# szpiech/garlic

Measured on AMD Instinct MI355X. Metric: LOD-windows/sec (SNPs x inds / winsize), higher is better.
Workload: dtype f64

## Files before the change

### garlic_amd/csrc/garlic_hip.hip

```cpp
#include "../../include/garlic_hip.h"
#include "lod_kernels.hpp"
#include "variant_kernels.hpp"
#include "ld_kernels.hpp"
#include "ld_multi_kernel.hpp"
#include "tgls_ring_kernel.hpp"
#include "tgls_wide_kernel.hpp"
#include "tgls_feed_kernel.hpp"
#include "tgls_feed_multi_kernel.hpp"
#include "wlod_strip_kernel.hpp"
#include "wlod_small_kernel.hpp"
#include "coverage_kernel.hpp"
#include "roh_segments_kernel.hpp"
#include "feed_kernel.hpp"
#include "wlod_feed_kernel.hpp"
#include "feed_sort_kernel.hpp"
#include "kde_kernels.hpp"
#include "kde_multi_kernels.hpp"
#include "kde_part_set_kernels.hpp"
#include "gmm_kernels.hpp"
#include "feature_kernels.hpp"
#include "../host/kde_select.hpp"
#include "../host/kde_parts.hpp"
#include "../host/chain_order.hpp"
#include "bed_kernels.hpp"
// ... 225 lines not shown
    {
        if (p) (void)score_free(ctx, p);
        p = nullptr;
    }
};


struct garlic_panel {
    garlic_ctx *ctx = nullptr;
    int32_t nchr = 0;
    int32_t nind = 0;
    int64_t nloci = 0;
    int64_t nind_pad = 0;
    int64_t nwordrows = 0;
    std::vector<int32_t> chr_nloci;
    std::vector<int64_t> chr_off;
    std::vector<int32_t> pos, cs, ce;
    std::vector<double> gpos, freq;
    bool have_map = false, have_freq = false, have_geno = false, have_gpos = false;
    DevBuf<uint32_t> d_packed;
    DevBuf<int32_t> d_pos, d_cs, d_ce;
    DevBuf<int64_t> d_chr_off;
    DevBuf<double> d_tab;
    bool tab_valid = false;
    double tab_error = 0;
    double tab_min = 0, tabgl_min = 0, glterms_min = 0;
    bool tab_all_finite = false;
    bool seg_valid = false;
    int32_t seg_max_gap = 0;
    std::vector<int64_t> boundaries;
    DevBuf<int32_t> d_blk_counts, d_blk_offsets, d_total;
    DevBuf<int64_t> d_boundaries;
    DevBuf<ChainItem> d_items;
    DevBuf<FeedItem> d_feed_items;
    DevBuf<FillItem> d_fill;
    DevBuf<int32_t> d_counter;
    DevBuf<ChrDev> d_chrs;
    DevBuf<int16_t> d_stage16;
    DevBuf<int32_t> d_bed_word_rows;
    DevBuf<int64_t> d_row_counts;
    bool have_gl = false;
    std::vector<double> gl_values;
    std::unordered_map<uint64_t, int> gl_code;
    DevBuf<uint8_t> d_codes;
    DevBuf<double> d_tabgl;
    bool tabgl_valid = false;
    DevBuf<double> d_glterms;
    bool glterms_valid = false, glterms_scaled = false;
    int32_t glterms_M = 0;
    double glterms_mu = 0.0;
    int64_t terms_budget = 0;
    DevBuf<double> d_slab[2];
    hipStream_t slab_stream = nullptr;
    hipEvent_t ev_slab_begin = nullptr, ev_slab_built[2] = {}, ev_slab_read[2] = {};
    DevBuf<int32_t> d_slab_queues;
    int32_t last_slab_blocks = 0, last_n_slabs = 0;

    int tabgl_ncodes = 0;
    bool gl_cont = false;
    DevBuf<double> d_glval;
    bool gl_vals_dropped = false;
    bool gl_cover_required = false;
    std::vector<uint8_t> gl_cover;
    DevBuf<double> d_freq;
    bool dfreq_valid = false;
    int gl_terms_by = 0;
// ... 1412 lines not shown
    const bool ring_patch = !getenv("GARLIC_WLOD_GL_NO_PATCH");
    const int strip_waves = (W + 15 - 16 * WS_WAVES <= 16 || getenv("GARLIC_WLOD_STRIP_NARROW_ONLY")) ? WS_WAVES : WS_WAVES_WIDE;
    const bool wlod_gl_strip = wlod_gl_ring && W + 15 - 16 * strip_waves <= 16 && !getenv("GARLIC_WLOD_GL_NO_STRIP");
    f.strip_waves = strip_waves;
    f.use_patch = wlod_gl_ring ? ring_patch : wlod_use_patch;
    f.tile_lds = wlod_gl_ring ? WLOD_GL_RING_OFF + (size_t)WLOD_WAVES * GARLIC_WLOD_GL_RING_ROWS * WAVE * 8
                              : wlod_rows + 16 + (wlod_use_patch ? wlod_patch : 0);
    f.strip_force_rerun = wlod_gl_strip && getenv("GARLIC_WLOD_STRIP_FORCE_RERUN") != nullptr;
    f.family = wlod_stream                            ? Family::wlod_stream
               : wlod_small                           ? Family::wlod_small_tiles
               : wlod_gl_strip                        ? Family::wlod_strip
               : wlod_gl_ring                         ? Family::wlod_glring
               : f.wlod_gl                            ? Family::wlod_tile_gl
               : !getenv("GARLIC_WLOD_ONE_BLOCK")     ? Family::wlod_tile2
                                                      : Family::wlod_tile;
    return GARLIC_OK;
}

void finish_form(const garlic_panel *p, const LodCall &c, const Layout &L, const double *d_out, LodForm &f)
{
    f.aligned16 = (c.pitch_align % 2 == 0) && ((reinterpret_cast<uintptr_t>(d_out) & 15) == 0);
    if (f.family == Family::wlod_stream && !f.aligned16) f.family = Family::wlod_small_tiles;
    f.strip_three = f.family == Family::wlod_strip && f.strip_waves != WS_WAVES_WIDE && f.aligned16 && !f.cov_bits &&
                    !getenv("GARLIC_WLOD_STRIP_TWO_PER_CU");
    for (int k = 0; f.strip_three && k < p->nchr; k++) f.strip_three = L.pitch[k] * 8 < ((int64_t)1 << 32);
}

using Plan = garlic_panel::Plan;

struct LodWork {
    std::vector<Run> runs;
    std::vector<FillItem> fill;
    std::vector<ChainItem> items;
    std::vector<FeedItem> feed_items;
    std::vector<ChrDev> chrs;
    std::vector<uint8_t> valid;
    std::vector<int2> tiles, segs;
    std::vector<WlodStrip> strips;
    std::vector<int32_t> feed_blocks;
};

int chain_workers(const garlic_ctx *ctx, size_t n_items)
{
    int workers = ctx->n_cu;
    if (const char *e = getenv("GARLIC_WORKERS")) workers = std::max(1, atoi(e));
    return std::min<int>(workers, (int)n_items);
}

int plan_lod(garlic_panel *p, const LodCall &c, const LodForm &form, const Layout &L, const garlic_panel::PlanKey &key, LodWork &w, Plan &plan)
{
    plan = Plan{false, key};
    const int nblk = (c.ind_count + WAVE - 1) / WAVE;
    int rc;
    p->plan.valid = false;
    plan_runs(p, c.W, w.runs, w.fill, plan.n_valid);
    const std::vector<int> order = longest_first(w.runs);
    w.items.reserve(w.runs.size() * nblk);
    const bool wlod_slabs = form.slab_blocks && (form.wlod_tuned || form.family == Family::wlod_feed);
    const int per_list = form.slab_blocks ? form.slab_blocks : std::max(nblk, 1);
    for (int k0 = 0; k0 < nblk && (!w.runs.empty() || wlod_slabs); ) {
        if (c.blocks && !(*c.blocks)[(size_t)k0]) { k0++; continue; }
        const int k1 = std::min(nblk, k0 + per_list);
        const size_t item0 = w.items.size();
        for (size_t i = 0; i < order.size(); i++) {
            const Run &r = w.runs[order[i]];
            for (int k = k0; k < k1; k++)
                if (!c.blocks || (*c.blocks)[(size_t)k]) w.items.push_back(ChainItem{r.chr, r.a, r.b, k * WAVE});
        }
        if (form.slab_blocks) plan.slabs.push_back(Plan::Slab{c.ind_begin / WAVE + k0, c.ind_begin / WAVE + k1, item0, w.items.size() - item0});
        k0 = k1;
    }
    if (form.family == Family::chain && !form.slab_blocks) {
        std::vector<int32_t> len(w.items.size());
        for (size_t i = 0; i < len.size(); i++) len[i] = w.items[i].b - w.items[i].a + 1;
        const std::vector<int> at = garlic_host::chainOrder(len, chain_workers(p->ctx, len.size()));
        std::vector<ChainItem> sorted(w.items.size());
        for (size_t i = 0; i < at.size(); i++) sorted[i] = w.items[(size_t)at[i]];
        w.items.swap(sorted);
    }
    if (form.family == Family::feed) {
        std::vector<int32_t> col0(w.runs.size());
        for (size_t i = 0; i < w.runs.size(); i++) {
            const int32_t s = (w.runs[i].a + c.thin_step - 1) / c.thin_step;
            col0[i] = (int64_t)s * c.thin_step <= w.runs[i].b ? s : -1;
        }
        build_feed_items(w.runs, order, c.blocks, nblk, col0, w.feed_items);
        plan.n_feed_items = w.feed_items.size();
    }
    w.chrs.resize(p->nchr);
    for (int k = 0; k < p->nchr; k++)
        w.chrs[k] = ChrDev{p->chr_off[k], L.base[k], L.pitch[k], p->chr_nloci[k],
                           (c.pitch_align >= 2 && 64 * L.pitch[k] * 8 + 512 < ((int64_t)1 << 32)) ? 1 : 0};
    plan.n_items = w.items.size();
    plan.n_fill = w.fill.size();
    plan.n_runs = (int64_t)w.runs.size();
    if (!p->d_counter.p) {
        if ((rc = p->d_counter.reserve(8))) return rc;
        HIP_TRY(hipMemsetAsync(p->d_counter.p, 0, 8 * sizeof(int32_t), p->ctx->stream));
    }
    if (form.wlod_tuned || form.family == Family::wlod_feed) {
        w.valid.assign((size_t)p->nloci, 0);
        for (const Run &r : w.runs)
            memset(w.valid.data() + p->chr_off[r.chr] + r.a, 1, (size_t)(r.b - r.a + 1));
    }
    if (form.family == Family::wlod_feed) {
        for (int k = 0; k < p->nchr; k++) {
            const int32_t cols = (int32_t)(((int64_t)p->chr_nloci[k] + c.thin_step - 1) / c.thin_step);
            for (int32_t c0 = 0; c0 < cols; c0 += WFD_COLS) w.tiles.push_back(make_int2(k, c0));
        }
        plan.n_tiles = (int32_t)w.tiles.size();
        for (int k = 0; k < nblk; k++)
            if (!c.blocks || (*c.blocks)[(size_t)k]) w.feed_blocks.push_back(k);
        plan.n_feed_blocks = (int32_t)w.feed_blocks.size();
        size_t at = 0;
        for (Plan::Slab &sl : plan.slabs) {
            sl.fb0 = (int32_t)at;
            while (at < w.feed_blocks.size() && w.feed_blocks[at] < sl.b1) at++;
            sl.n_fb = (int32_t)at - sl.fb0;
        }
    }
    if (form.wlod_tuned) {
        for (int k = 0; k < p->nchr; k++)
            for (int s0 = 0; s0 < p->chr_nloci[k]; s0 += TILE) w.tiles.push_back(make_int2(k, s0));
        plan.n_tiles = (int32_t)w.tiles.size();
        for (int k = 0; k < p->nchr; k++)
// ... 157 lines not shown
        HIP_TRY(hipLaunchKernel(fn, dim3((sa.n_work + 7u) / 8u * 8u), dim3((form.strip_waves + 1) * WAVE), kargs, strip_lds, s));
        if (form.strip_force_rerun) HIP_TRY(hipMemsetAsync(p->d_counter.p + 3, 1, sizeof(int32_t), s));
        a.run_if = p->d_counter.p + 3;
        a.rerun_count = p->d_counter.p + 4;
        p->reruns_stale = true;
    }
    const void *fn = wlod_tile_fn(form.family, form.wlod_gl, form.aligned16);
    if (form.tile_lds > LDS_DEFAULT_MAX) HIP_TRY(hipFuncSetAttribute(fn, hipFuncAttributeMaxDynamicSharedMemorySize, (int)form.tile_lds));
    void *kargs[] = {(void *)&a_packed, (void *)&a_wtab, (void *)&a_skew, (void *)&d_out, (void *)&a};
    HIP_TRY(hipLaunchKernel(fn, dim3((a.n_work + 7u) / 8u * 8u), wl_block, kargs, form.tile_lds, s));
    return GARLIC_OK;
}

bool chain_takes_fill(const LodForm &form, const Plan &plan, Family family)
{
    return family == Family::chain && plan.n_items && plan.n_fill && !form.wlod_tuned && !form.cov_bits;
}

int launch_chain(garlic_panel *p, const LodCall &c, const LodForm &form, Plan &plan, const LodWork *fresh, int workers, double *d_out)
{
    garlic_ctx *ctx = p->ctx;
    ItemTrace trace;
    if (form.family == Family::feed && plan.n_feed_items) {
        FeedArgs f{p->d_packed.p, p->d_tab.p, p->d_feed_items.p, p->d_chrs.p, d_out, nullptr, p->nwordrows, c.ind_begin, c.ind_count, c.W,
                   (int32_t)plan.n_feed_items, c.thin_step, form.feed_asm ? 1 : 0, p->d_counter.p, nullptr};
        f.trace = trace.begin(8, plan.n_feed_items, "\n", ctx->stream);
        int grid = (int)std::min<size_t>(plan.n_feed_items, (size_t)ctx->n_cu * std::max(1, plan.feed_per_cu)), rc;
        if (fresh && (rc = feed_grid(ctx, fresh->feed_items, &grid, &plan.feed_per_cu))) return rc;
        void *kargs[] = {(void *)&f};
        HIP_TRY(hipLaunchKernel((const void *)lod_feed_kernel, dim3((unsigned)grid), dim3(FEED_G * WAVE), kargs, 0, ctx->stream));
    } else {
        ChainArgs a{p->d_packed.p, p->d_tab.p, p->d_items.p,     p->d_chrs.p,          d_out, p->nind_pad, p->nwordrows,
                    c.ind_begin,   c.ind_count, c.W,             (int32_t)plan.n_items, p->d_counter.p, nullptr,
                    nullptr,       0};
        if (chain_takes_fill(form, plan, form.family)) {
            a.fill = p->d_fill.p;
            a.n_fill = (int32_t)plan.n_fill;
        }
        a.trace = trace.begin(4, plan.n_items, " 0\n", ctx->stream);
        if (form.aligned16)
            hipLaunchKernelGGL((lod_chain_kernel<true>), dim3((unsigned)workers), dim3(CHAIN_THREADS), 0, ctx->stream, a);
        else
            hipLaunchKernelGGL((lod_chain_kernel<false>), dim3((unsigned)workers), dim3(CHAIN_THREADS), 0, ctx->stream, a);
    }
    trace.write(ctx->stream);
    return GARLIC_OK;
}

template <class Chains>
int for_each_tgls_slab(garlic_panel *p, const std::vector<Plan::Slab> &slabs, int32_t slab_blocks, Chains chains, bool scaled = false)
{
    garlic_ctx *ctx = p->ctx;
    hipStream_t s = ctx->stream;
    const int64_t rows = GOFF + p->nloci + GPAD_BACK;
    const size_t n_slabs = slabs.size();
    int rc;
    p->last_slab_blocks = slab_blocks;
    p->last_n_slabs = (int32_t)n_slabs;
    if (!n_slabs) return GARLIC_OK;
    if (!p->slab_stream) {
        HIP_TRY(hipStreamCreateWithFlags(&p->slab_stream, hipStreamNonBlocking));
        for (hipEvent_t *ev : {&p->ev_slab_begin, &p->ev_slab_built[0], &p->ev_slab_built[1], &p->ev_slab_read[0], &p->ev_slab_read[1]})
            HIP_TRY(hipEventCreateWithFlags(ev, hipEventDisableTiming));
    }
    for (int q = 0; q < 2; q++) {
        size_t blocks = 0;
        for (size_t k = (size_t)q; k < n_slabs; k += 2) blocks = std::max(blocks, (size_t)(slabs[k].b1 - slabs[k].b0));
// ... 114 lines not shown
    return GARLIC_OK;
}

int launch_wlod_feed(garlic_panel *p, const LodCall &c, const LodForm &form, const Plan &plan, double *d_out, const WlodTerms &t,
                     int32_t fb0, int32_t n_fb)
{
    const int nquad = (n_fb + WFD_WAVES - 1) / WFD_WAVES;
    WlodFeedArgs a{p->d_packed.p, form.wlod_gl ? t.terms : p->d_wtab.p, p->d_skew.p + SKEW_FRONT, p->d_valid.p, p->d_chrs.p,
                   p->d_tiles.p, p->d_feed_blocks.p + fb0, d_out, p->nwordrows, GOFF + p->nloci + GPAD_BACK, c.ind_count, c.W, c.thin_step,
                   n_fb, nquad, (uint32_t)((int64_t)plan.n_tiles * nquad), t.blk0};
    if (!a.n_work) return GARLIC_OK;
    if (form.wlod_gl) hipLaunchKernelGGL(wlod_feed_kernel<true>, dim3(a.n_work), dim3(WFD_WAVES * WAVE), 0, p->ctx->stream, a);
    else hipLaunchKernelGGL(wlod_feed_kernel<false>, dim3(a.n_work), dim3(WFD_WAVES * WAVE), 0, p->ctx->stream, a);
    return GARLIC_OK;
}

int launch_wlod_slabs(garlic_panel *p, const LodCall &c, const LodForm &form, const Plan &plan, double *d_out)
{
    return for_each_tgls_slab(p, plan.slabs, form.slab_blocks, [&](size_t k, const double *terms) {
        const Plan::Slab &sl = plan.slabs[k];
        const WlodTerms t = wlod_terms_slab(c, sl, terms);
        if (form.family == Family::wlod_feed) return launch_wlod_feed(p, c, form, plan, d_out, t, sl.fb0, sl.n_fb);
        return launch_wlod(p, c, form, plan, d_out, t);
    }, true);
}

int enqueue_lod(garlic_panel *p, const LodCall &c, const LodForm &form, const Layout &L, Plan &plan, const LodWork *fresh,
                double *d_out, Family family, bool one_kernel = false)
{
    garlic_ctx *ctx = p->ctx;
    hipStream_t s = ctx->stream;
    int rc = GARLIC_OK;
    if (!one_kernel) HIP_TRY(hipEventRecord(ctx->ev_begin, s));
    if (fresh && ((rc = p->d_chrs.put(fresh->chrs, s)) || (rc = p->d_items.put(fresh->items, s)) || (rc = p->d_fill.put(fresh->fill, s)) ||
                  (rc = p->d_feed_items.put(fresh->feed_items, s)) || (rc = p->d_valid.put(fresh->valid, s)) ||
                  (rc = p->d_tiles.put(fresh->tiles, s)) || (rc = p->d_segs.put(fresh->segs, s)) || (rc = p->d_strips.put(fresh->strips, s)) ||
                  (rc = p->d_feed_blocks.put(fresh->feed_blocks, s))))
        return rc;
    if (family == Family::feed || family == Family::tgls_feed) {
        hipLaunchKernelGGL(fill_value_kernel, dim3(1024), dim3(256), 0, s, d_out, L.total, MISSING_D);
    } else if (plan.n_fill && !form.wlod_tuned && family != Family::wlod_feed && !form.cov_bits &&
               !chain_takes_fill(form, plan, family)) {
        dim3 grid((unsigned)plan.n_fill, (unsigned)((c.ind_count + FILL_ROWS - 1) / FILL_ROWS));
        hipLaunchKernelGGL(fill_missing_kernel, grid, dim3(256), 0, s, p->d_fill.p, p->d_chrs.p, c.ind_count, d_out);
    }
    if (plan.n_items && (fresh || c.mode != MODE_LOD)) HIP_TRY(hipMemsetAsync(p->d_counter.p, 0, 2 * sizeof(int32_t), s));
    p->stats_slot = (int)(ctx->n_calls % garlic_ctx::HIST);
    HIP_TRY(hist_mark(ctx, false));
    const int workers = chain_workers(ctx, plan.n_items);
    if (form.wlod_tuned || plan.n_items || family == Family::wlod_feed)
        switch (family) {
        case Family::chain:
        case Family::feed: rc = launch_chain(p, c, form, plan, fresh, workers, d_out); break;
        case Family::exact:
            hipLaunchKernelGGL(lod_chain_exact_kernel, dim3((unsigned)plan.n_items), dim3(WAVE), 0, s, variant_args(p, c, form, d_out),
                               (int)plan.n_items);
            break;
        case Family::tgls_ring:
        case Family::tgls_feed:
        case Family::tgls_terms:
        case Family::tgls_lookup: rc = launch_tgls(p, c, form, plan, workers, d_out); break;
        case Family::wlod_generic: rc = launch_generic_wlod(p, c, form, plan, d_out); break;
        case Family::wlod_feed:
            rc = form.slab_blocks ? launch_wlod_slabs(p, c, form, plan, d_out)
                                  : launch_wlod_feed(p, c, form, plan, d_out, wlod_terms_whole(p, c), 0, plan.n_feed_blocks);
            break;
        default:
// ... 5186 lines not shown
```

### garlic_amd/csrc/lod_kernels.hpp

```cpp
#pragma once
#include <hip/hip_runtime.h>
#include <stdint.h>

#include "chain_loop_gfx950.inc"

namespace garlic {

constexpr int WAVE = 64;
constexpr int TILE = 32;
constexpr int TPITCH = 34;
constexpr int GOFF = 32;
constexpr int GPAD_CHAIN = 32 * GARLIC_CHAIN_NSLOT + 48 * GARLIC_CHAIN_CHROWS + 64;
constexpr int GPAD_BACK = GPAD_CHAIN > 4160 ? GPAD_CHAIN : 4160;
constexpr double MISSING_D = -9999.0;

struct ChrDev {
    int64_t loc_base;
    int64_t out_base;
    int64_t out_pitch;
    int32_t nloci;
    int32_t fast;
};

struct ChainItem {
    int32_t chr;
    int32_t a;
    int32_t b;
    int32_t ind0;
};

struct FillItem {
    int32_t chr;
    int32_t lo;
    int32_t hi;
    int32_t pad;
};

__device__ __host__ __forceinline__ int64_t packed_index(int64_t w, int64_t col, int64_t nwordrows)
{
    return (((col >> 6) * nwordrows + w) << 6) + (col & 63);
}

__global__ void pack_genotypes_kernel(const int16_t *__restrict__ geno, int64_t ld,
                                      int64_t locus_begin, int64_t locus_count, int32_t nind,
                                      int64_t nind_pad, int64_t nwordrows,
                                      uint32_t *__restrict__ packed, int64_t word_lo,
                                      int64_t word_hi)
{
    int64_t ind = (int64_t)blockIdx.x * blockDim.x + threadIdx.x;
    int64_t w = word_lo + blockIdx.y;
    if (ind >= nind_pad || w >= word_hi) return;
    uint32_t *dst = packed + packed_index(w, ind, nwordrows);
    uint32_t word = *dst;
    if (ind >= nind) { *dst = 0xFFFFFFFFu; return; }
    int64_t g0 = w * 16 - GOFF;
#pragma unroll
    for (int q = 0; q < 16; q++) {
        int64_t l = g0 + q - locus_begin;
        if (l >= 0 && l < locus_count) {
            int v = geno[l * ld + ind];
            uint32_t code = (v == 0) ? 0u : (v == 1) ? 1u : (v == 2) ? 2u : 3u;
            word = (word & ~(3u << (2 * q))) | (code << (2 * q));
// ... 139 lines not shown
__device__ __forceinline__ void fill_rows(const FillItem &it, const ChrDev &c, int row0, int32_t nind, double *out,
                                          int wave, int nwaves, int lane)
{
    for (int r = row0 + wave; r < row0 + FILL_ROWS && r < nind; r += nwaves) {
        double *row = out + c.out_base + (int64_t)r * c.out_pitch;
        for (int l = it.lo + lane; l < it.hi; l += WAVE) row[l] = MISSING_D;
    }
}

__global__ void __launch_bounds__(256)
fill_missing_kernel(const FillItem *items, const ChrDev *chrs, int32_t nind, double *out)
{
    FillItem it = items[blockIdx.x];
    ChrDev c = chrs[it.chr];
    fill_rows(it, c, blockIdx.y * FILL_ROWS, nind, out, threadIdx.x >> 6, 4, threadIdx.x & 63);
}

struct ChainArgs {
    const uint32_t *packed;
    const double *tab;
    const ChainItem *items;
    const ChrDev *chrs;
    double *out;
    int64_t nind_pad;
    int64_t nwordrows;
    int32_t ind_begin;
    int32_t ind_count;
    int32_t winsize;
    int32_t n_items;
    int32_t *next_item;
    int64_t *trace;
    const FillItem *fill;
    int32_t n_fill;
};

__device__ __forceinline__ void chain_fill_share(const ChainArgs &p, int wave, int first, int lane)
{
    const int groups = (p.ind_count + FILL_ROWS - 1) / FILL_ROWS;
    const int64_t units = (int64_t)p.n_fill * groups;
    for (int64_t u = blockIdx.x; u < units; u += gridDim.x) {
        const FillItem it = p.fill[u / groups];
        const ChrDev c = p.chrs[it.chr];
        fill_rows(it, c, (int)(u % groups) * FILL_ROWS, p.ind_count, p.out, wave - first, 4 - first, lane);
    }
}

constexpr uint32_t SLOT_BYTES = 3072;
constexpr uint32_t SL_LW1 = 0, SL_LW2 = 256, SL_TW1 = 512, SL_TW2 = 768;
constexpr uint32_t SL_LTAB = 1024, SL_TTAB = 2048;
constexpr uint32_t LDS_ITEM = 3072;
constexpr uint32_t LDS_TILE = GARLIC_CHAIN_LDS_TILE0;
constexpr uint32_t LDS_BYTES = GARLIC_CHAIN_LDS_TOTAL;
constexpr int CHAIN_THREADS = 256;

struct Streams {
    int64_t lead_w, trail_w;
    const double *lead_tab, *trail_tab;
    int sh_lead, sh_trail;
};

__device__ __forceinline__ void advance(Streams &st)
{
    st.lead_w += 2; st.trail_w += 2;
    st.lead_tab += 4 * TILE; st.trail_tab += 4 * TILE;
}

__device__ __forceinline__ void fill_regs(unsigned char *smem, const Streams &st,
                                          const uint32_t *gcol, int lane)
{
    const uint32_t l1 = gcol[(st.lead_w + 1) * WAVE], l2 = gcol[(st.lead_w + 2) * WAVE];
    const uint32_t t1 = gcol[(st.trail_w + 1) * WAVE], t2 = gcol[(st.trail_w + 2) * WAVE];
    const double2 tl = reinterpret_cast<const double2 *>(st.lead_tab)[lane];
    const double2 tt = reinterpret_cast<const double2 *>(st.trail_tab)[lane];
    *reinterpret_cast<uint32_t *>(smem + SL_LW1 + lane * 4) = l1;
    *reinterpret_cast<uint32_t *>(smem + SL_LW2 + lane * 4) = l2;
    *reinterpret_cast<uint32_t *>(smem + SL_TW1 + lane * 4) = t1;
    *reinterpret_cast<uint32_t *>(smem + SL_TW2 + lane * 4) = t2;
    *reinterpret_cast<double2 *>(smem + SL_LTAB + lane * 16) = tl;
    *reinterpret_cast<double2 *>(smem + SL_TTAB + lane * 16) = tt;
}

struct TileBits {
    uint32_t lead_lo, lead_hi, trail_lo, trail_hi;
};

template <int SLOT>
__device__ __forceinline__ TileBits tile_consume(const unsigned char *smem, uint32_t &lc,
                                                 uint32_t &tc, const Streams &st, int lane)
{
    const unsigned char *slot = smem + SLOT * SLOT_BYTES;
    const uint32_t l1 = *reinterpret_cast<const uint32_t *>(slot + SL_LW1 + lane * 4);
    const uint32_t l2 = *reinterpret_cast<const uint32_t *>(slot + SL_LW2 + lane * 4);
    const uint32_t t1 = *reinterpret_cast<const uint32_t *>(slot + SL_TW1 + lane * 4);
    const uint32_t t2 = *reinterpret_cast<const uint32_t *>(slot + SL_TW2 + lane * 4);
    TileBits tb;
    tb.lead_lo = __builtin_amdgcn_alignbit(l1, lc, st.sh_lead);
    tb.lead_hi = __builtin_amdgcn_alignbit(l2, l1, st.sh_lead);
    tb.trail_lo = __builtin_amdgcn_alignbit(t1, tc, st.sh_trail);
    tb.trail_hi = __builtin_amdgcn_alignbit(t2, t1, st.sh_trail);
    lc = l2;
    tc = t2;
    return tb;
}

template <bool EDGE, int SLOT>
__device__ __forceinline__ void tile_steps(const unsigned char *smem, unsigned char *tile,
                                           double &acc, const TileBits &tb, int s0, int a, int b,
                                           int lane)
{
    const unsigned char *slot = smem + SLOT * SLOT_BYTES;
    const uint32_t tile_lane = (uint32_t)lane * (TPITCH * 8);
#pragma unroll
// ... 10 lines not shown
            if (!(s >= a && s <= b)) t_in = 0.0;
        }
        acc = (acc - t_out) + t_in;
        *reinterpret_cast<double *>(tile + tile_lane + j * 8) = acc;
    }
}

template <bool EDGE, bool ALIGNED16>
__device__ __forceinline__ void tile_store(const unsigned char *tile, int s0, int a, int b, int lane,
                                           int rows_valid, double *out_tile, int64_t pitch)
{
    const int rsub = lane >> 4, csub = lane & 15;
#pragma unroll
    for (int q = 0; q < WAVE / 4; q++) {
        const int qe = (4 * q < rows_valid) ? q : 0;
        const int re = min(rsub, rows_valid - 1 - 4 * qe);
        const double2 v = *reinterpret_cast<const double2 *>(
            tile + (uint32_t)(4 * qe + re) * (TPITCH * 8) + csub * 16);
        char *base = reinterpret_cast<char *>(out_tile + (int64_t)(4 * qe) * pitch);
        const uint32_t off = (uint32_t)re * (uint32_t)(pitch * 8) + (uint32_t)csub * 16u;
        double *dst = reinterpret_cast<double *>(base + off);
        if (EDGE) {
            const int s = s0 + 2 * csub;
            if (s >= a && s <= b) dst[0] = v.x;
            if (s + 1 >= a && s + 1 <= b) dst[1] = v.y;
        } else if (!ALIGNED16) {
            dst[0] = v.x;
            dst[1] = v.y;
        } else {
            *reinterpret_cast<double2 *>(dst) = v;
        }
    }
}

__global__ void __launch_bounds__(256) fill_value_kernel(double *dst, int64_t n, double value)
{
    for (int64_t i = (int64_t)blockIdx.x * blockDim.x + threadIdx.x; i < n; i += (int64_t)gridDim.x * blockDim.x)
        dst[i] = value;
}

template <bool ALIGNED16>
__global__ void __launch_bounds__(CHAIN_THREADS)
lod_chain_kernel(ChainArgs p)
{
    __shared__ __attribute__((aligned(16))) unsigned char smem[LDS_BYTES];
    unsigned char *tile = smem + LDS_TILE;
    const int lane = threadIdx.x & (WAVE - 1);
    const int wave = __builtin_amdgcn_readfirstlane(threadIdx.x >> 6);
    bool fill_pending = p.n_fill > 0;
    for (;;) {
    if (threadIdx.x == 0)
        *reinterpret_cast<int *>(smem + LDS_ITEM) = atomicAdd(p.next_item, 1);
    __syncthreads();
    const int item_idx =
        __builtin_amdgcn_readfirstlane(*reinterpret_cast<const int *>(smem + LDS_ITEM));
    __syncthreads();
    if (item_idx >= p.n_items) {
        if (fill_pending) chain_fill_share(p, wave, 0, lane);
        if (threadIdx.x == 0) {
            __threadfence();
            if (atomicAdd(p.next_item + 1, 1) == (int)gridDim.x - 1) {
                p.next_item[0] = 0;
                p.next_item[1] = 0;
            }
        }
        return;
    }
    if (p.trace && threadIdx.x == 0) {
        p.trace[4 * item_idx + 0] = blockIdx.x;
        p.trace[4 * item_idx + 1] = wall_clock64();
    }
    if (fill_pending) {
        if (wave != 0) chain_fill_share(p, wave, 1, lane);
        fill_pending = false;
    }
    const ChainItem it = p.items[item_idx];
    const ChrDev c = p.chrs[it.chr];
    const int W = p.winsize;
    const int a = it.a, b = it.b;
    const int rows_valid = min(WAVE, p.ind_count - it.ind0);
    const int64_t col0 = (int64_t)p.ind_begin + it.ind0;
    const uint32_t *gcol = p.packed + packed_index(0, col0 + lane, p.nwordrows);
    const int64_t Gbase = c.loc_base + GOFF;

    double acc = 0.0;
    if (wave == 0) {
        int l = a;
        const int lend = a + W - 1;
        while (l < lend) {
            const int64_t G = Gbase + l;
            const int sh = 2 * (int)(G & 15);
            const uint32_t *wp = gcol + (G >> 4) * WAVE;
            uint32_t wd[5];
#pragma unroll
            for (int q = 0; q < 5; q++) wd[q] = wp[q * WAVE];
            uint32_t al[4];
#pragma unroll
            for (int q = 0; q < 4; q++) al[q] = __builtin_amdgcn_alignbit(wd[q + 1], wd[q], sh);
            const int n = min(64, lend - l);
            double t[64];
#pragma unroll
            for (int q = 0; q < 64; q++) {
                const uint32_t g = (al[q >> 4] >> (2 * (q & 15))) & 3u;
                t[q] = p.tab[(G + min(q, n - 1)) * 4 + ((q < n) ? g : 3u)];
            }
#pragma unroll
            for (int q = 0; q < 64; q++) acc += (q < n) ? t[q] : 0.0;
            l += n;
        }
    }

    int s0 = a & ~(TILE - 1);
    Streams st;
    {
        const int64_t Glead = Gbase + s0 + W - 1;
        const int64_t Gtrail = Gbase + s0 - 1;
        st.sh_lead = 2 * (int)(Glead & 15);
        st.sh_trail = 2 * (int)(Gtrail & 15);
        st.lead_w = Glead >> 4;
        st.trail_w = Gtrail >> 4;
        st.lead_tab = p.tab + Glead * 4;
        st.trail_tab = p.tab + Gtrail * 4;
    }
    double *const out_row = p.out + c.out_base + (int64_t)it.ind0 * c.out_pitch;
    double *out_tile = out_row + s0;
    const int64_t pitch = c.out_pitch;

    for (int phase = 0; phase < 2; phase++) {
        const int last = (phase == 0) ? s0 : b;
        while (s0 <= last && s0 <= b) {
            if (wave == 0) {
                uint32_t lc = gcol[st.lead_w * WAVE];
                uint32_t tc = gcol[st.trail_w * WAVE];
                fill_regs(smem, st, gcol, lane);
                const TileBits tb = tile_consume<0>(smem, lc, tc, st, lane);
                tile_steps<true, 0>(smem, tile, acc, tb, s0, a, b, lane);
                tile_store<true, ALIGNED16>(tile, s0, a, b, lane, rows_valid, out_tile, pitch);
            }
            advance(st);
            s0 += TILE;
            out_tile += TILE;
        }
        if (phase == 1 || !ALIGNED16 || !c.fast || (col0 & 63) != 0) continue;
        if (st.lead_w - st.trail_w > GARLIC_CHAIN_MAX_DW) continue;

        int ntiles = (b + 1 - s0) / TILE;
        if (ntiles >= 2) {
            uint32_t lc = gcol[st.lead_w * WAVE];
            uint32_t tc = gcol[st.trail_w * WAVE];
            const int64_t chunk0 = st.trail_w / GARLIC_CHAIN_CHROWS;
            const int64_t chunkI = (st.lead_w + 2 * GARLIC_CHAIN_NSLOT) / GARLIC_CHAIN_CHROWS + 1;
            const uint32_t *pchunk =
                p.packed + packed_index(GARLIC_CHAIN_CHROWS * chunk0, col0, p.nwordrows);
            const uint32_t wmask = GARLIC_CHAIN_WROWS - 1;
            if (p.trace && threadIdx.x == 0) p.trace[4 * item_idx + 2] = wall_clock64();
            const uint32_t a_nchunk0 = (uint32_t)(chunkI - chunk0 + 1) * (GARLIC_CHAIN_CHROWS / 4);
            const uint32_t a_roff0 = (uint32_t)((GARLIC_CHAIN_CHROWS * chunk0) & wmask) * 256u;
            const uint32_t a_laddr0 = (uint32_t)(st.lead_w & wmask) * 256u;
            const uint32_t a_taddr0 = (uint32_t)(st.trail_w & wmask) * 256u;
            if (wave == 0) {
                uint32_t tin[4], tout[4];
#pragma unroll
                for (int q = 0; q < 4; q++) {
                    const uint32_t bb = 4u * (uint32_t)lane + (uint32_t)q;
                    const uint32_t sp = (bb & 3u) | (((bb >> 2) & 3u) << 8) | (((bb >> 4) & 3u) << 16) | (((bb >> 6) & 3u) << 24);
                    tin[q] = sp << 4;
                    tout[q] = sp << 6;
                }
                *reinterpret_cast<uint4 *>(smem + GARLIC_CHAIN_SPREAD_IN + lane * 16) = make_uint4(tin[0], tin[1], tin[2], tin[3]);
                *reinterpret_cast<uint4 *>(smem + GARLIC_CHAIN_SPREAD_OUT + lane * 16) = make_uint4(tout[0], tout[1], tout[2], tout[3]);
            }
            {
                asm volatile(GARLIC_CHAIN_LOOP_ASM
                             : [acc] "+v"(acc)
                             : [wave] "s"(wave), [lane] "v"(lane), [lc] "v"(lc), [tc] "v"(tc),
                               [pchunk] "s"(pchunk), [nchunk0] "s"(a_nchunk0), [roff0] "s"(a_roff0),
                               [laddr0] "s"(a_laddr0), [taddr0] "s"(a_taddr0),
                               [pltab] "s"(st.lead_tab), [pttab] "s"(st.trail_tab), [out] "s"(out_tile),
                               [ntiles] "s"(ntiles), [shl] "s"(st.sh_lead), [sht] "s"(st.sh_trail),
                               [pitch8] "s"((uint32_t)(pitch * 8)), [rows] "s"(rows_valid)
                             : GARLIC_CHAIN_LOOP_CLOBBERS);
            }
            st.lead_w += 2 * ntiles;
            st.trail_w += 2 * ntiles;
            st.lead_tab += (int64_t)(4 * TILE) * ntiles;
            st.trail_tab += (int64_t)(4 * TILE) * ntiles;
            s0 += ntiles * TILE;
            out_tile += (int64_t)ntiles * TILE;
            __syncthreads();
        }
    }
    if (p.trace && threadIdx.x == 0) p.trace[4 * item_idx + 3] = wall_clock64();
    }
}

}
```

Baseline: 7.546 billion.

## Prefetch chain item metadata and overlap head window sum with loop setup

Each chain item and its chromosome record are packed on the host into one 48-byte ChainWork record. The kernel reads it with three vector loads plus readfirstlane, replacing two dependent loads. The head-of-window LOD sum now loads all packed words up front and gathers in 64-wide batches with lookahead. Meanwhile the other waves prefetch the asm loop's first column words and build the spread tables. The first tile's loads are also issued before the head gather so their latency hides behind it. This restructures control flow and adds a __syncthreads and register pressure, with a risk of divergence bugs in the tile loop.

```diff
diff --git a/garlic_amd/csrc/garlic_hip.hip b/garlic_amd/csrc/garlic_hip.hip
--- a/garlic_amd/csrc/garlic_hip.hip
+++ b/garlic_amd/csrc/garlic_hip.hip
@@ -281,6 +281,7 @@
     DevBuf<int32_t> d_blk_counts, d_blk_offsets, d_total;
     DevBuf<int64_t> d_boundaries;
     DevBuf<ChainItem> d_items;
+    DevBuf<ChainWork> d_work;
     DevBuf<FeedItem> d_feed_items;
     DevBuf<FillItem> d_fill;
     DevBuf<int32_t> d_counter;
@@ -1759,6 +1760,7 @@
     std::vector<Run> runs;
     std::vector<FillItem> fill;
     std::vector<ChainItem> items;
+    std::vector<ChainWork> work;
     std::vector<FeedItem> feed_items;
     std::vector<ChrDev> chrs;
     std::vector<uint8_t> valid;
@@ -1818,6 +1820,7 @@
     for (int k = 0; k < p->nchr; k++)
         w.chrs[k] = ChrDev{p->chr_off[k], L.base[k], L.pitch[k], p->chr_nloci[k],
                            (c.pitch_align >= 2 && 64 * L.pitch[k] * 8 + 512 < ((int64_t)1 << 32)) ? 1 : 0};
+    if (form.family == Family::chain || form.family == Family::feed) w.work = chainWork(w.items, w.chrs);
     plan.n_items = w.items.size();
     plan.n_fill = w.fill.size();
     plan.n_runs = (int64_t)w.runs.size();
@@ -2041,7 +2044,7 @@
     } else {
         ChainArgs a{p->d_packed.p, p->d_tab.p, p->d_items.p,     p->d_chrs.p,          d_out, p->nind_pad, p->nwordrows,
                     c.ind_begin,   c.ind_count, c.W,             (int32_t)plan.n_items, p->d_counter.p, nullptr,
-                    nullptr,       0};
+                    nullptr,       0,           p->d_work.p};
         if (chain_takes_fill(form, plan, form.family)) {
             a.fill = p->d_fill.p;
             a.n_fill = (int32_t)plan.n_fill;
@@ -2222,7 +2225,8 @@
     hipStream_t s = ctx->stream;
     int rc = GARLIC_OK;
     if (!one_kernel) HIP_TRY(hipEventRecord(ctx->ev_begin, s));
-    if (fresh && ((rc = p->d_chrs.put(fresh->chrs, s)) || (rc = p->d_items.put(fresh->items, s)) || (rc = p->d_fill.put(fresh->fill, s)) ||
+    if (fresh && ((rc = p->d_chrs.put(fresh->chrs, s)) || (rc = p->d_items.put(fresh->items, s)) || (rc = p->d_work.put(fresh->work, s)) ||
+                  (rc = p->d_fill.put(fresh->fill, s)) ||
                   (rc = p->d_feed_items.put(fresh->feed_items, s)) || (rc = p->d_valid.put(fresh->valid, s)) ||
                   (rc = p->d_tiles.put(fresh->tiles, s)) || (rc = p->d_segs.put(fresh->segs, s)) || (rc = p->d_strips.put(fresh->strips, s)) ||
                   (rc = p->d_feed_blocks.put(fresh->feed_blocks, s))))
diff --git a/garlic_amd/csrc/lod_kernels.hpp b/garlic_amd/csrc/lod_kernels.hpp
--- a/garlic_amd/csrc/lod_kernels.hpp
+++ b/garlic_amd/csrc/lod_kernels.hpp
@@ -3,6 +3,7 @@
 #include <stdint.h>
 
 #include "chain_loop_gfx950.inc"
+#include "../host/chain_work.hpp"
 
 namespace garlic {
 
@@ -14,20 +15,6 @@
 constexpr int GPAD_BACK = GPAD_CHAIN > 4160 ? GPAD_CHAIN : 4160;
 constexpr double MISSING_D = -9999.0;
 
-struct ChrDev {
-    int64_t loc_base;
-    int64_t out_base;
-    int64_t out_pitch;
-    int32_t nloci;
-    int32_t fast;
-};
-
-struct ChainItem {
-    int32_t chr;
-    int32_t a;
-    int32_t b;
-    int32_t ind0;
-};
 
 struct FillItem {
     int32_t chr;
@@ -233,6 +220,7 @@
     int64_t *trace;
     const FillItem *fill;
     int32_t n_fill;
+    const ChainWork *work;
 };
 
 __device__ __forceinline__ void chain_fill_share(const ChainArgs &p, int wave, int first, int lane)
@@ -266,19 +254,33 @@
     st.lead_tab += 4 * TILE; st.trail_tab += 4 * TILE;
 }
 
-__device__ __forceinline__ void fill_regs(unsigned char *smem, const Streams &st,
-                                          const uint32_t *gcol, int lane)
-{
-    const uint32_t l1 = gcol[(st.lead_w + 1) * WAVE], l2 = gcol[(st.lead_w + 2) * WAVE];
-    const uint32_t t1 = gcol[(st.trail_w + 1) * WAVE], t2 = gcol[(st.trail_w + 2) * WAVE];
-    const double2 tl = reinterpret_cast<const double2 *>(st.lead_tab)[lane];
-    const double2 tt = reinterpret_cast<const double2 *>(st.trail_tab)[lane];
-    *reinterpret_cast<uint32_t *>(smem + SL_LW1 + lane * 4) = l1;
-    *reinterpret_cast<uint32_t *>(smem + SL_LW2 + lane * 4) = l2;
-    *reinterpret_cast<uint32_t *>(smem + SL_TW1 + lane * 4) = t1;
-    *reinterpret_cast<uint32_t *>(smem + SL_TW2 + lane * 4) = t2;
-    *reinterpret_cast<double2 *>(smem + SL_LTAB + lane * 16) = tl;
-    *reinterpret_cast<double2 *>(smem + SL_TTAB + lane * 16) = tt;
+struct TileLoads {
+    uint32_t lc, tc, l1, l2, t1, t2;
+    double2 tl, tt;
+};
+
+__device__ __forceinline__ TileLoads tile_request(const Streams &st, const uint32_t *gcol, int lane)
+{
+    TileLoads r;
+    r.lc = gcol[st.lead_w * WAVE];
+    r.tc = gcol[st.trail_w * WAVE];
+    r.l1 = gcol[(st.lead_w + 1) * WAVE];
+    r.l2 = gcol[(st.lead_w + 2) * WAVE];
+    r.t1 = gcol[(st.trail_w + 1) * WAVE];
+    r.t2 = gcol[(st.trail_w + 2) * WAVE];
+    r.tl = reinterpret_cast<const double2 *>(st.lead_tab)[lane];
+    r.tt = reinterpret_cast<const double2 *>(st.trail_tab)[lane];
+    return r;
+}
+
+__device__ __forceinline__ void slot_put(unsigned char *smem, const TileLoads &r, int lane)
+{
+    *reinterpret_cast<uint32_t *>(smem + SL_LW1 + lane * 4) = r.l1;
+    *reinterpret_cast<uint32_t *>(smem + SL_LW2 + lane * 4) = r.l2;
+    *reinterpret_cast<uint32_t *>(smem + SL_TW1 + lane * 4) = r.t1;
+    *reinterpret_cast<uint32_t *>(smem + SL_TW2 + lane * 4) = r.t2;
+    *reinterpret_cast<double2 *>(smem + SL_LTAB + lane * 16) = r.tl;
+    *reinterpret_cast<double2 *>(smem + SL_TTAB + lane * 16) = r.tt;
 }
 
 struct TileBits {
@@ -355,6 +357,43 @@
         }
     }
 }
+
+__device__ __forceinline__ void head_gather(double (&t)[64], const double *tab, int64_t G, const uint32_t *wd, int sh)
+{
+    uint32_t al[4];
+#pragma unroll
+    for (int q = 0; q < 4; q++) al[q] = __builtin_amdgcn_alignbit(wd[q + 1], wd[q], sh);
+    const double *row = tab + G * 4;
+#pragma unroll
+    for (int q = 0; q < 64; q++) {
+        const uint32_t g = (al[q >> 4] >> (2 * (q & 15))) & 3u;
+        t[q] = row[q * 4 + g];
+    }
+}
+
+__device__ __forceinline__ void head_add(double &acc, const double (&t)[64], int n)
+{
+#pragma unroll
+    for (int q = 0; q < 64; q++) acc += (q < n) ? t[q] : 0.0;
+}
+
+__device__ __forceinline__ ChainWork load_work(const ChainWork *w)
+{
+    const uint4 *q = reinterpret_cast<const uint4 *>(w);
+    const uint4 q0 = q[0], q1 = q[1], q2 = q[2];
+    const auto u = [](uint32_t v) { return (uint32_t)__builtin_amdgcn_readfirstlane((int)v); };
+    const auto u64 = [&](uint32_t lo, uint32_t hi) { return (int64_t)(((uint64_t)u(hi) << 32) | u(lo)); };
+    ChainWork r;
+    r.it = ChainItem{(int32_t)u(q0.x), (int32_t)u(q0.y), (int32_t)u(q0.z), (int32_t)u(q0.w)};
+    r.loc_base = u64(q1.x, q1.y);
+    r.out_base = u64(q1.z, q1.w);
+    r.out_pitch = u64(q2.x, q2.y);
+    r.fast = (int32_t)u(q2.z);
+    r.pad = 0;
+    return r;
+}
+
+constexpr int HEAD_WORDS = 9;
 
 __global__ void __launch_bounds__(256) fill_value_kernel(double *dst, int64_t n, double value)
 {
@@ -397,41 +436,13 @@
         if (wave != 0) chain_fill_share(p, wave, 1, lane);
         fill_pending = false;
     }
-    const ChainItem it = p.items[item_idx];
-    const ChrDev c = p.chrs[it.chr];
+    const ChainWork cw = load_work(p.work + item_idx);
     const int W = p.winsize;
-    const int a = it.a, b = it.b;
-    const int rows_valid = min(WAVE, p.ind_count - it.ind0);
-    const int64_t col0 = (int64_t)p.ind_begin + it.ind0;
+    const int a = cw.it.a, b = cw.it.b;
+    const int rows_valid = min(WAVE, p.ind_count - cw.it.ind0);
+    const int64_t col0 = (int64_t)p.ind_begin + cw.it.ind0;
     const uint32_t *gcol = p.packed + packed_index(0, col0 + lane, p.nwordrows);
-    const int64_t Gbase = c.loc_base + GOFF;
-
-    double acc = 0.0;
-    if (wave == 0) {
-        int l = a;
-        const int lend = a + W - 1;
-        while (l < lend) {
-            const int64_t G = Gbase + l;
-            const int sh = 2 * (int)(G & 15);
-            const uint32_t *wp = gcol + (G >> 4) * WAVE;
-            uint32_t wd[5];
-#pragma unroll
-            for (int q = 0; q < 5; q++) wd[q] = wp[q * WAVE];
-            uint32_t al[4];
-#pragma unroll
-            for (int q = 0; q < 4; q++) al[q] = __builtin_amdgcn_alignbit(wd[q + 1], wd[q], sh);
-            const int n = min(64, lend - l);
-            double t[64];
-#pragma unroll
-            for (int q = 0; q < 64; q++) {
-                const uint32_t g = (al[q >> 4] >> (2 * (q & 15))) & 3u;
-                t[q] = p.tab[(G + min(q, n - 1)) * 4 + ((q < n) ? g : 3u)];
-            }
-#pragma unroll
-            for (int q = 0; q < 64; q++) acc += (q < n) ? t[q] : 0.0;
-            l += n;
-        }
-    }
+    const int64_t Gbase = cw.loc_base + GOFF;
 
     int s0 = a & ~(TILE - 1);
     Streams st;
@@ -445,73 +456,118 @@
         st.lead_tab = p.tab + Glead * 4;
         st.trail_tab = p.tab + Gtrail * 4;
     }
-    double *const out_row = p.out + c.out_base + (int64_t)it.ind0 * c.out_pitch;
+    double *const out_row = p.out + cw.out_base + (int64_t)cw.it.ind0 * cw.out_pitch;
     double *out_tile = out_row + s0;
-    const int64_t pitch = c.out_pitch;
-
-    for (int phase = 0; phase < 2; phase++) {
-        const int last = (phase == 0) ? s0 : b;
-        while (s0 <= last && s0 <= b) {
-            if (wave == 0) {
-                uint32_t lc = gcol[st.lead_w * WAVE];
-                uint32_t tc = gcol[st.trail_w * WAVE];
-                fill_regs(smem, st, gcol, lane);
-                const TileBits tb = tile_consume<0>(smem, lc, tc, st, lane);
-                tile_steps<true, 0>(smem, tile, acc, tb, s0, a, b, lane);
-                tile_store<true, ALIGNED16>(tile, s0, a, b, lane, rows_valid, out_tile, pitch);
+    const int64_t pitch = cw.out_pitch;
+
+    const int ntiles = (b + 1 - (s0 + TILE)) / TILE;
+    const bool loop = ALIGNED16 && cw.fast && (col0 & 63) == 0 && st.lead_w - st.trail_w <= GARLIC_CHAIN_MAX_DW && ntiles >= 2;
+
+    double acc = 0.0;
+    uint32_t lc = 0, tc = 0;
+    if (wave != 0) {
+        if (loop) {
+            lc = gcol[(st.lead_w + 2) * WAVE];
+            tc = gcol[(st.trail_w + 2) * WAVE];
+        }
+    } else {
+        const int nt = W - 1;
+        const int64_t G0 = Gbase + a;
+        const int sh = 2 * (int)(G0 & 15);
+        const uint32_t *wp = gcol + (G0 >> 4) * WAVE;
+        uint32_t wd[HEAD_WORDS];
+#pragma unroll
+        for (int q = 0; q < HEAD_WORDS; q++) wd[q] = wp[q * WAVE];
+        const TileLoads head = tile_request(st, gcol, lane);
+        if (nt <= 128) {
+            double t0[64], t1[64];
+            head_gather(t0, p.tab, G0, wd, sh);
+            if (nt > 64) head_gather(t1, p.tab, G0 + 64, wd + 4, sh);
+            head_add(acc, t0, min(64, nt));
+            if (nt > 64) head_add(acc, t1, nt - 64);
+        } else {
+            uint32_t cur[5], nxt[5];
+#pragma unroll
+            for (int q = 0; q < 5; q++) { cur[q] = wd[q]; nxt[q] = wd[q + 4]; }
+            for (int l = 0; l < nt; l += 64) {
+                uint32_t ahead[5];
+#pragma unroll
+                for (int q = 0; q < 5; q++) ahead[q] = wp[(l / 16 + 8 + q) * WAVE];
+                const int n = min(64, nt - l);
+                double t[64];
+                head_gather(t, p.tab, G0 + l, cur, sh);
+                head_add(acc, t, n);
+#pragma unroll
+                for (int q = 0; q < 5; q++) { cur[q] = nxt[q]; nxt[q] = ahead[q]; }
             }
-            advance(st);
-            s0 += TILE;
-            out_tile += TILE;
-        }
-        if (phase == 1 || !ALIGNED16 || !c.fast || (col0 & 63) != 0) continue;
-        if (st.lead_w - st.trail_w > GARLIC_CHAIN_MAX_DW) continue;
-
-        int ntiles = (b + 1 - s0) / TILE;
-        if (ntiles >= 2) {
-            uint32_t lc = gcol[st.lead_w * WAVE];
-            uint32_t tc = gcol[st.trail_w * WAVE];
-            const int64_t chunk0 = st.trail_w / GARLIC_CHAIN_CHROWS;
-            const int64_t chunkI = (st.lead_w + 2 * GARLIC_CHAIN_NSLOT) / GARLIC_CHAIN_CHROWS + 1;
-            const uint32_t *pchunk =
-                p.packed + packed_index(GARLIC_CHAIN_CHROWS * chunk0, col0, p.nwordrows);
-            const uint32_t wmask = GARLIC_CHAIN_WROWS - 1;
-            if (p.trace && threadIdx.x == 0) p.trace[4 * item_idx + 2] = wall_clock64();
-            const uint32_t a_nchunk0 = (uint32_t)(chunkI - chunk0 + 1) * (GARLIC_CHAIN_CHROWS / 4);
-            const uint32_t a_roff0 = (uint32_t)((GARLIC_CHAIN_CHROWS * chunk0) & wmask) * 256u;
-            const uint32_t a_laddr0 = (uint32_t)(st.lead_w & wmask) * 256u;
-            const uint32_t a_taddr0 = (uint32_t)(st.trail_w & wmask) * 256u;
-            if (wave == 0) {
-                uint32_t tin[4], tout[4];
-#pragma unroll
-                for (int q = 0; q < 4; q++) {
-                    const uint32_t bb = 4u * (uint32_t)lane + (uint32_t)q;
-                    const uint32_t sp = (bb & 3u) | (((bb >> 2) & 3u) << 8) | (((bb >> 4) & 3u) << 16) | (((bb >> 6) & 3u) << 24);
-                    tin[q] = sp << 4;
-                    tout[q] = sp << 6;
-                }
-                *reinterpret_cast<uint4 *>(smem + GARLIC_CHAIN_SPREAD_IN + lane * 16) = make_uint4(tin[0], tin[1], tin[2], tin[3]);
-                *reinterpret_cast<uint4 *>(smem + GARLIC_CHAIN_SPREAD_OUT + lane * 16) = make_uint4(tout[0], tout[1], tout[2], tout[3]);
+        }
+        slot_put(smem, head, lane);
+        lc = head.lc;
+        tc = head.tc;
+        const TileBits tb = tile_consume<0>(smem, lc, tc, st, lane);
+        tile_steps<true, 0>(smem, tile, acc, tb, s0, a, b, lane);
+    }
+    if (loop) {
+        __syncthreads();
+        if (wave == 1) {
+            uint32_t tin[4], tout[4];
+#pragma unroll
+            for (int q = 0; q < 4; q++) {
+                const uint32_t bb = 4u * (uint32_t)lane + (uint32_t)q;
+                const uint32_t sp = (bb & 3u) | (((bb >> 2) & 3u) << 8) | (((bb >> 4) & 3u) << 16) | (((bb >> 6) & 3u) << 24);
+                tin[q] = sp << 4;
+                tout[q] = sp << 6;
             }
-            {
-                asm volatile(GARLIC_CHAIN_LOOP_ASM
-                             : [acc] "+v"(acc)
-                             : [wave] "s"(wave), [lane] "v"(lane), [lc] "v"(lc), [tc] "v"(tc),
-                               [pchunk] "s"(pchunk), [nchunk0] "s"(a_nchunk0), [roff0] "s"(a_roff0),
-                               [laddr0] "s"(a_laddr0), [taddr0] "s"(a_taddr0),
-                               [pltab] "s"(st.lead_tab), [pttab] "s"(st.trail_tab), [out] "s"(out_tile),
-                               [ntiles] "s"(ntiles), [shl] "s"(st.sh_lead), [sht] "s"(st.sh_trail),
-                               [pitch8] "s"((uint32_t)(pitch * 8)), [rows] "s"(rows_valid)
-                             : GARLIC_CHAIN_LOOP_CLOBBERS);
-            }
-            st.lead_w += 2 * ntiles;
-            st.trail_w += 2 * ntiles;
-            st.lead_tab += (int64_t)(4 * TILE) * ntiles;
-            st.trail_tab += (int64_t)(4 * TILE) * ntiles;
-            s0 += ntiles * TILE;
-            out_tile += (int64_t)ntiles * TILE;
-            __syncthreads();
-        }
+            *reinterpret_cast<uint4 *>(smem + GARLIC_CHAIN_SPREAD_IN + lane * 16) = make_uint4(tin[0], tin[1], tin[2], tin[3]);
+            *reinterpret_cast<uint4 *>(smem + GARLIC_CHAIN_SPREAD_OUT + lane * 16) = make_uint4(tout[0], tout[1], tout[2], tout[3]);
+        }
+    }
+    if (wave == 0) tile_store<true, ALIGNED16>(tile, s0, a, b, lane, rows_valid, out_tile, pitch);
+    advance(st);
+    s0 += TILE;
+    out_tile += TILE;
+
+    if (loop) {
+        const int64_t chunk0 = st.trail_w / GARLIC_CHAIN_CHROWS;
+        const int64_t chunkI = (st.lead_w + 2 * GARLIC_CHAIN_NSLOT) / GARLIC_CHAIN_CHROWS + 1;
+        const uint32_t *pchunk =
+            p.packed + packed_index(GARLIC_CHAIN_CHROWS * chunk0, col0, p.nwordrows);
+        const uint32_t wmask = GARLIC_CHAIN_WROWS - 1;
+        if (p.trace && threadIdx.x == 0) p.trace[4 * item_idx + 2] = wall_clock64();
+        const uint32_t a_nchunk0 = (uint32_t)(chunkI - chunk0 + 1) * (GARLIC_CHAIN_CHROWS / 4);
+        const uint32_t a_roff0 = (uint32_t)((GARLIC_CHAIN_CHROWS * chunk0) & wmask) * 256u;
+        const uint32_t a_laddr0 = (uint32_t)(st.lead_w & wmask) * 256u;
+        const uint32_t a_taddr0 = (uint32_t)(st.trail_w & wmask) * 256u;
+        asm volatile(GARLIC_CHAIN_LOOP_ASM
+                     : [acc] "+v"(acc)
+                     : [wave] "s"(wave), [lane] "v"(lane), [lc] "v"(lc), [tc] "v"(tc),
+                       [pchunk] "s"(pchunk), [nchunk0] "s"(a_nchunk0), [roff0] "s"(a_roff0),
+                       [laddr0] "s"(a_laddr0), [taddr0] "s"(a_taddr0),
+                       [pltab] "s"(st.lead_tab), [pttab] "s"(st.trail_tab), [out] "s"(out_tile),
+                       [ntiles] "s"(ntiles), [shl] "s"(st.sh_lead), [sht] "s"(st.sh_trail),
+                       [pitch8] "s"((uint32_t)(pitch * 8)), [rows] "s"(rows_valid)
+                     : GARLIC_CHAIN_LOOP_CLOBBERS);
+        st.lead_w += 2 * ntiles;
+        st.trail_w += 2 * ntiles;
+        st.lead_tab += (int64_t)(4 * TILE) * ntiles;
+        st.trail_tab += (int64_t)(4 * TILE) * ntiles;
+        s0 += ntiles * TILE;
+        out_tile += (int64_t)ntiles * TILE;
+        __syncthreads();
+    }
+    while (s0 <= b) {
+        if (wave == 0) {
+            const TileLoads r = tile_request(st, gcol, lane);
+            slot_put(smem, r, lane);
+            lc = r.lc;
+            tc = r.tc;
+            const TileBits tb = tile_consume<0>(smem, lc, tc, st, lane);
+            tile_steps<true, 0>(smem, tile, acc, tb, s0, a, b, lane);
+            tile_store<true, ALIGNED16>(tile, s0, a, b, lane, rows_valid, out_tile, pitch);
+        }
+        advance(st);
+        s0 += TILE;
+        out_tile += TILE;
     }
     if (p.trace && threadIdx.x == 0) p.trace[4 * item_idx + 3] = wall_clock64();
     }
diff --git a/garlic_amd/host/chain_work.hpp b/garlic_amd/host/chain_work.hpp
--- /dev/null
+++ b/garlic_amd/host/chain_work.hpp
@@ -0,0 +1,44 @@
+#pragma once
+#include <stddef.h>
+#include <stdint.h>
+
+#include <vector>
+
+namespace garlic {
+
+struct ChrDev {
+    int64_t loc_base;
+    int64_t out_base;
+    int64_t out_pitch;
+    int32_t nloci;
+    int32_t fast;
+};
+
+struct ChainItem {
+    int32_t chr;
+    int32_t a;
+    int32_t b;
+    int32_t ind0;
+};
+
+struct ChainWork {
+    ChainItem it;
+    int64_t loc_base;
+    int64_t out_base;
+    int64_t out_pitch;
+    int32_t fast;
+    int32_t pad;
+};
+static_assert(sizeof(ChainWork) == 48, "three 16-byte pieces, no holes");
+
+inline std::vector<ChainWork> chainWork(const std::vector<ChainItem> &items, const std::vector<ChrDev> &chrs)
+{
+    std::vector<ChainWork> work(items.size());
+    for (size_t i = 0; i < items.size(); i++) {
+        const ChrDev c = items[i].chr >= 0 ? chrs[(size_t)items[i].chr] : ChrDev{};
+        work[i] = ChainWork{items[i], c.loc_base, c.out_base, c.out_pitch, c.fast, 0};
+    }
+    return work;
+}
+
+}
```

Measured after the change: 7.539 billion. Within noise of the previous version (-0.1%).
